# Harshs27/uGLAD

Measured on AMD Instinct MI355X. Metric: GLAD unroll-steps/sec (batch D×D Θ-updates), M=1024 D=128 L=30, higher is better.
Workload: dtype f32; 1 GPU; multi-task M=1024/GPU D=128 L=30 fp32 (BASELINE config 3; global batch 1024); pass=training step: forward + loss + backward + gradient exchange + Adam, sqrt_mode=ns10, parallelism=batch-sharded x1

## Files before the change

### uglad_amd/csrc/cell_bwd.h

```cpp
template <int NT>
__global__ __launch_bounds__(kThreads) void UGLAD_CELL_BWD_NAME(
    const float* __restrict__ Gnext, const float* __restrict__ S, const float* __restrict__ Zin,
    const float* __restrict__ half, const float* __restrict__ U, const float* __restrict__ beta,
    const float* __restrict__ lam_ptr, const float* __restrict__ params, float* __restrict__ Gout,
    float* __restrict__ grad_rho_partial, float* __restrict__ glam_partial, float* __restrict__ gws, int D, int mode,
#if UGLAD_CELL_BWD_GS
    int gs, int k_count, int lam_stride, float* __restrict__ gS) {
#else
    int gs, int k_count, int lam_stride) {
#endif
  constexpr int DP = NT * 32, LD = DP + 1;
  UGLAD_BIG_BUFFERS(sX, DP * LD, sY, DP * LD, gws)
  __shared__ float s_beta[DP], s_r[DP];
  __shared__ __attribute__((aligned(16))) float s_a0[DP], s_aN[DP];
  __shared__ float s_red[8];
  __shared__ float s_g[kWaves][kNRho + 1];
  const int tid = threadIdx.x, lane = tid & 63, w = tid >> 6;
  const size_t base = (size_t)blockIdx.x * D * D;
  const float* Sm = S + base;
  const float* Gm = Gnext + base;
  float* Go = Gout + base;
  const int grp = blockIdx.x / gs;
  params += (size_t)grp * kNParam;
  const size_t step_mdd = (size_t)gridDim.x * D * D, step_md = (size_t)gridDim.x * D;
  float g[kNRho];
#pragma unroll
  for (int q = 0; q < kNRho; ++q) g[q] = 0.f;
  constexpr int kMaxQ = ((DP / 2) * (DP + 1) + kThreads - 1) / kThreads;
  constexpr bool kPre = DP <= 128;
  constexpr int kQ = kPre ? kMaxQ : 8;
  constexpr int kIShift = kPre ? 8 : 16, kJMask = (1 << kIShift) - 1;
  const int D1 = D + 1, total = ((D + 1) / 2) * D1;
  const int sp = kThreads / D1, sc = kThreads - sp * D1;
  auto entry = [&](int e, int p, int c) -> int {
    if (e >= total) return -1;
    if (c < D - p) return (p << kIShift) | (p + c);
    const int i = D - 1 - p;
    return (i == p) ? -1 : ((i << kIShift) | (i + (c - (D - p))));
  };
  auto advance = [&](int& p, int& c) {
    c += sc;
    p += sp;
    if (c >= D1) {
      c -= D1;
      ++p;
    }
  };
  __shared__ unsigned short s_ent[kPre ? kMaxQ : 1][kPre ? kThreads : 1];
  if constexpr (kPre) {
    int p = tid / D1, c = tid - p * D1;
    for (int q = 0; q < kMaxQ; ++q) {
      s_ent[q][tid] = (unsigned short)entry(tid + kThreads * q, p, c);
      advance(p, c);
    }
  }
#pragma unroll 1
  for (int s = 0; s < k_count; ++s) {
    const bool first = (s == 0), last = (s == k_count - 1);
    const int tid = opaque_v(threadIdx.x), lane = tid & 63;
    const int w = __builtin_amdgcn_readfirstlane(tid >> 6);
    const float* Zm = Zin + base - s * step_mdd;
    const float* Hm = half + base - s * step_mdd;
    const float* Um = U + base - s * step_mdd;
    const float* bm = beta + (size_t)blockIdx.x * D - s * step_md;
    const float lam = lam_ptr[(long)grp - (long)s * lam_stride];
    const float c4 = 4.0f / lam, inv_lam2 = 1.0f / (lam * lam);

    KSTAMP(0);
    constexpr int kV4 = DP * DP / 4, kC4 = DP / 4;
    constexpr bool kFull4 = kV4 % (8 * kThreads) == 0, kFull1 = (DP * DP) % (8 * kThreads) == 0;
    const bool vec16 = (D == DP) && (((reinterpret_cast<size_t>(U) | (first ? reinterpret_cast<size_t>(Gnext) : 0)) & 15) == 0);
    if (vec16) {
      if (first) {
        for (int v0 = 0; v0 < kV4; v0 += 8 * kThreads) {
          f4 u[8], gv[8];
#pragma unroll
          for (int q = 0; q < 8; ++q) {
            const int idx = v0 + q * kThreads + tid;
            const unsigned at = (kFull4 || idx < kV4) ? 16u * idx : 0u;
            u[q] = load_at<f4>(Um, at);
            gv[q] = load_at<f4>(Gm, at);
          }
#pragma unroll
          for (int q = 0; q < 8; ++q) {
            const int idx = v0 + q * kThreads + tid;
            if (kFull4 || idx < kV4) {
              const int i = idx / kC4, k = 4 * (idx - i * kC4);
              sX[i * LD + k] = u[q].x, sX[i * LD + k + 1] = u[q].y, sX[i * LD + k + 2] = u[q].z, sX[i * LD + k + 3] = u[q].w;
              sY[i * LD + k] = gv[q].x, sY[i * LD + k + 1] = gv[q].y, sY[i * LD + k + 2] = gv[q].z, sY[i * LD + k + 3] = gv[q].w;
            }
          }
        }
      } else {
        for (int v0 = 0; v0 < kV4; v0 += 8 * kThreads) {
          f4 u[8];
#pragma unroll
          for (int q = 0; q < 8; ++q) {
            const int idx = v0 + q * kThreads + tid;
            u[q] = load_at<f4>(Um, (kFull4 || idx < kV4) ? 16u * idx : 0u);
          }
#pragma unroll
          for (int q = 0; q < 8; ++q) {
            const int idx = v0 + q * kThreads + tid;
            if (kFull4 || idx < kV4) {
              const int i = idx / kC4, k = 4 * (idx - i * kC4);
              sX[i * LD + k] = u[q].x, sX[i * LD + k + 1] = u[q].y, sX[i * LD + k + 2] = u[q].z, sX[i * LD + k + 3] = u[q].w;
            }
          }
        }
      }
    } else {
      constexpr int si = kThreads / DP, sk = kThreads - si * DP;
      int i = tid / DP, k = tid - i * DP;
      int off = i * D + k;
      const int soff = si * D + sk, wrap = D - DP;
      if (first) {
        for (int idx0 = 0; idx0 < DP * DP; idx0 += 8 * kThreads) {
          float u[8], gv[8];
          int dst[8];
          bool in[8];
#pragma unroll
          for (int q = 0; q < 8; ++q) {
            in[q] = (kFull1 || idx0 + q * kThreads + tid < DP * DP) && i < D && k < D;
            const unsigned at = in[q] ? 4u * off : 0u;
            u[q] = load_at<float>(Um, at);
            gv[q] = load_at<float>(Gm, at);
            dst[q] = i * LD + k;
            i += si, k += sk, off += soff;
            if (k >= DP) k -= DP, ++i, off += wrap;
          }
          __builtin_amdgcn_sched_barrier(0);
#pragma unroll
          for (int q = 0; q < 8; ++q) {
            if (kFull1 || idx0 + q * kThreads + tid < DP * DP) {
              sX[dst[q]] = in[q] ? u[q] : 0.f;
              sY[dst[q]] = in[q] ? gv[q] : 0.f;
            }
          }
        }
      } else {
        for (int idx0 = 0; idx0 < DP * DP; idx0 += 8 * kThreads) {
          float u[8];
          int dst[8];
          bool in[8];
#pragma unroll
          for (int q = 0; q < 8; ++q) {
            in[q] = (kFull1 || idx0 + q * kThreads + tid < DP * DP) && i < D && k < D;
            u[q] = load_at<float>(Um, in[q] ? 4u * off : 0u);
            dst[q] = i * LD + k;
            i += si, k += sk, off += soff;
            if (k >= DP) k -= DP, ++i, off += wrap;
          }
          __builtin_amdgcn_sched_barrier(0);
#pragma unroll
          for (int q = 0; q < 8; ++q) {
            if (kFull1 || idx0 + q * kThreads + tid < DP * DP) sX[dst[q]] = in[q] ? u[q] : 0.f;
          }
        }
      }
    }
    float a2 = 0.f;
    if (tid < D) {
      const float be = bm[tid];
      const float al = fmaf(be, be, c4);
      a2 = al * al;
    }
    const float nrmA = sqrtf(block_sum(a2, s_red));
    float r2 = 0.f;
    if (tid < DP) {
      float be = 0.f, r = 1.f;
      if (tid < D) {
        be = bm[tid];
        r = sqrt_spectrum(be, c4, nrmA, mode);
        r2 = r * r;
      }
      s_beta[tid] = be;
      s_r[tid] = r;
    }
    const float nrmR = sqrtf(block_sum(r2, s_red));
    if (mode == UGLAD_SQRT_NS10 && tid < DP) {
      float a = s_r[tid] / nrmR;
      s_a0[tid] = a;
#pragma unroll
      for (int it = 0; it < kNsIters; ++it) a = 0.5f * a * (3.f - a * a);
      s_aN[tid] = a;
    }
    __syncthreads();

    KSTAMP(1);
    using TU = Tiles<NT, true>;
    [[maybe_unused]] const int p0 = tid / D1, c0 = tid - p0 * D1;
    float gz[kQ];
    {
      [[maybe_unused]] int p = p0, c = c0;
      for (int q0 = 0; q0 < kMaxQ; q0 += kQ) {
        int pk[kQ];
        float hx[kQ], zz[kQ], gn[kQ], sv[kQ];
        if constexpr (kPre) {
#pragma unroll
          for (int u = 0; u < kQ; ++u) pk[u] = (int)(short)s_ent[u][tid];
          float gt[kQ];
#pragma unroll
          for (int u = 0; u < kQ; ++u) {
            const int i = pk[u] >> kIShift, j = pk[u] & kJMask;
            const bool in = pk[u] >= 0;
            const unsigned at = in ? 4u * ((unsigned)i * (unsigned)D + (unsigned)j) : 0u;
            gz[u] = 0.f;
            hx[u] = load_at<float>(Hm, at);
            zz[u] = load_at<float>(Zm, at);
            sv[u] = load_at<float>(Sm, at);
            gn[u] = sY[opaque_v(in ? i * LD + j : 0)];
            gt[u] = sY[opaque_v(in ? j * LD + i : 0)];
          }
#pragma unroll
          for (int u = 0; u < kQ; ++u) {
            const int i = pk[u] >> kIShift, j = pk[u] & kJMask;
            const bool in = pk[u] >= 0;
            hx[u] = in ? hx[u] : 0.f;
            zz[u] = in ? zz[u] : 0.f;
            sv[u] = in ? sv[u] : 0.f;
            gn[u] = in ? ((i == j) ? gn[u] : 0.5f * (gn[u] + gt[u])) : 0.f;
          }
        } else {
#pragma unroll
          for (int u = 0; u < kQ; ++u) {
            pk[u] = (q0 + u < kMaxQ) ? entry(tid + kThreads * (q0 + u), p, c) : -1;
            advance(p, c);
            const int i = pk[u] >> kIShift, j = pk[u] & kJMask;
            const bool in = pk[u] >= 0;
            hx[u] = in ? Hm[i * D + j] : 0.f;
            zz[u] = in ? Zm[i * D + j] : 0.f;
            sv[u] = in ? Sm[i * D + j] : 0.f;
            gn[u] = in ? ((i == j) ? sY[i * LD + j] : 0.5f * (sY[i * LD + j] + sY[j * LD + i])) : 0.f;
          }
        }
        constexpr int kQ2 = (kQ + 1) / 2;
#pragma unroll
        for (int h = 0; h < kQ2; ++h) {
          const int u0 = 2 * h, u1 = (2 * h + 1 < kQ) ? 2 * h + 1 : 2 * h;
          const bool has1 = 2 * h + 1 < kQ;
          if (!has1 && pk[u0] < 0) continue;
          RhoAct2 act2;
          rho_forward2(params, (v2f){hx[u0], has1 ? hx[u1] : 0.f}, (v2f){sv[u0], has1 ? sv[u1] : 0.f},
                       (v2f){zz[u0], has1 ? zz[u1] : 0.f}, act2);
#pragma unroll
          for (int c2 = 0; c2 < 2; ++c2) {
            const int u = c2 ? u1 : u0;
            if ((c2 == 0 || has1) && pk[u] >= 0) {
              const int i = pk[u] >> kIShift, j = pk[u] & kJMask;
              const RhoAct act = act2.half(c2);
              const float x = hx[u];
              const bool active = fabsf(x) > act.rho;
              const float sgn = (x > 0.f) ? 1.f : ((x < 0.f) ? -1.f : 0.f);
              const float g_rho = active ? -sgn * gn[u] : 0.f;
              float gx1, gx3;
              rho_backward(params, x, sv[u], zz[u], act, g_rho, (i == j) ? 1.f : 2.f, g, gx1, gx3);
#if UGLAD_CELL_BWD_GS
              gS[base + i * D + j] += rho_backward_col(params, act, g_rho, 1);
#endif
              const float gh = (active ? gn[u] : 0.f) + gx1;
              sY[i * LD + j] = gh;
              sY[j * LD + i] = gh;
              if (kPre) gz[u] = gx3;
              else Go[i * D + j] = gx3;
            }
          }
        }
      }
    }
    __syncthreads();

    KSTAMP(2);
    using T = Tiles<NT, false>;
    {
      f32x16 acc[T::kPerWave];
      gemm_lds<NT, false, false, false>(sY, sX, acc);
      __syncthreads();
      store_tiles<NT>(sY, acc);
    }
    __syncthreads();
    KSTAMP(3);
    float glam = 0.f;
    {
      f32x16 acc[TU::kPerWave];
      gemm_lds<NT, true, false, true>(sX, sY, acc);
      __syncthreads();
      KSTAMP(4);
#pragma unroll
      for (int n = 0; n < TU::kPerWave; ++n) {
        const int t = w + kWaves * n;
        if (t < TU::kCount) {
          int I, J;
          TU::ij(t, I, J);
          const int j = J * 32 + (lane & 31);
          const float a0j = s_a0[j], aNj = s_aN[j];
          const float rj = s_r[j], bj = s_beta[j];
          const float inv_2nrmR = 1.0f / (2.f * nrmR);
#pragma unroll
          for (int e4 = 0; e4 < 4; ++e4) {
            const int i0 = I * 32 + 8 * e4 + 4 * (lane >> 5);
            float Kr[4];
            if (mode == UGLAD_SQRT_EXACT) {
#pragma unroll
              for (int r = 0; r < 4; ++r) Kr[r] = 1.0f / (s_r[i0 + r] + rj);
            } else {
              const f4 a0 = *reinterpret_cast<const f4*>(&s_a0[i0]);
              const f4 aN = *reinterpret_cast<const f4*>(&s_aN[i0]);
              Kr[0] = ns_divided_difference(a0.x, a0j, aN.x, aNj, inv_2nrmR);
              Kr[1] = ns_divided_difference(a0.y, a0j, aN.y, aNj, inv_2nrmR);
              Kr[2] = ns_divided_difference(a0.z, a0j, aN.z, aNj, inv_2nrmR);
              Kr[3] = ns_divided_difference(a0.w, a0j, aN.w, aNj, inv_2nrmR);
            }
#pragma unroll
            for (int r = 0; r < 4; ++r) {
              const int e = 4 * e4 + r, i = i0 + r;
              if (I < J || i <= j) {
                float v = 0.f;
                if (i < D && j < D) {
                  const float K = Kr[r];
                  const float cij = acc[n][e];
                  if (i == j) glam = fmaf(cij, -2.f * K * inv_lam2, glam);
                  v = cij * 0.5f * fmaf(s_beta[i] + bj, K, -1.f);
                }
                sY[i * LD + j] = v;
                sY[j * LD + i] = v;
              }
            }
          }
        }
      }
    }
    __syncthreads();
    KSTAMP(5);
    {
      f32x16 acc[T::kPerWave];
      gemm_lds<NT, false, false, false>(sX, sY, acc);
      __syncthreads();
      store_tiles<NT>(sY, acc);
    }
    __syncthreads();
    KSTAMP(6);
    {
      f32x16 acc[TU::kPerWave];
      gemm_lds<NT, false, true, true>(sY, sX, acc);
      KSTAMP(7);
      __syncthreads();
#pragma unroll
      for (int n = 0; n < TU::kPerWave; ++n) {
        const int t = w + kWaves * n;
        if (t < TU::kCount) {
          int I, J;
          TU::ij(t, I, J);
#pragma unroll
          for (int e = 0; e < 16; ++e) sY[(I * 32 + acc_row(e, lane)) * LD + J * 32 + (lane & 31)] = acc[n][e];
        }
      }
    }
    __syncthreads();
    KSTAMP(20);
    {
      [[maybe_unused]] int p = p0, c = c0;
      for (int q0 = 0; q0 < kMaxQ; q0 += kQ) {
        int pk[kQ];
        float gb[kQ], sij[kQ];
#pragma unroll
        for (int u = 0; u < kQ; ++u) {
          if constexpr (kPre) {
            pk[u] = (int)(short)s_ent[u][tid];
          } else {
            pk[u] = (q0 + u < kMaxQ) ? entry(tid + kThreads * (q0 + u), p, c) : -1;
            advance(p, c);
          }
          const bool in = pk[u] >= 0;
          const int i = pk[u] >> kIShift, j = pk[u] & kJMask;
          gb[u] = sY[in ? i * LD + j : 0];
          sij[u] = load_at<float>(Sm, in ? 4u * ((unsigned)i * (unsigned)D + (unsigned)j) : 0u);
        }
        if (kPre) {
#pragma unroll
          for (int u = 0; u < kQ; ++u) {
            const bool in = pk[u] >= 0;
            const int i = pk[u] >> kIShift, j = pk[u] & kJMask;
            const float o = gz[u] - gb[u];
            sY[in ? i * LD + j : DP] = o;
            sY[in ? j * LD + i : DP] = o;
            glam = fmaf(in ? -sij[u] * inv_lam2 * ((i == j) ? 1.f : 2.f) : 0.f, gb[u], glam);
          }
        } else {
#pragma unroll
          for (int u = 0; u < kQ; ++u) {
            if (pk[u] >= 0) {
              const int i = pk[u] >> kIShift, j = pk[u] & kJMask;
              const float o = Go[i * D + j] - gb[u];
              sY[i * LD + j] = o;
              sY[j * LD + i] = o;
              glam = fmaf(-sij[u] * inv_lam2 * ((i == j) ? 1.f : 2.f), gb[u], glam);
            }
          }
        }
#if UGLAD_CELL_BWD_GS
        {
          const float inv_lam = 1.0f / lam;
#pragma unroll
          for (int u = 0; u < kQ; ++u) {
            if (pk[u] >= 0) {
              const int i = pk[u] >> kIShift, j = pk[u] & kJMask;
              const float v = fmaf(gb[u], inv_lam, gS[base + i * D + j]);
              gS[base + i * D + j] = v;
              gS[base + j * D + i] = v;
            }
          }
        }
#endif
      }
    }
    __syncthreads();
    KSTAMP(21);
    if (last) {
      const int si = kThreads / D, sj = kThreads - si * D;
      int i = tid / D, j = tid - i * D;
      for (int idx = tid; idx < D * D; idx += kThreads) {
        Go[idx] = sY[i * LD + j];
        j += sj;
        i += si;
        if (j >= D) {
          j -= D;
          ++i;
        }
      }
    }
    KSTAMP(8);
    if (last) {
#pragma unroll
      for (int q = 0; q < kNRho; ++q) {
        const float v = wave_sum(g[q]);
        if (lane == 0) s_g[w][q] = v;
      }
    }
    {
      const float v = wave_sum(glam);
      if (lane == 0) s_g[w][kNRho] = v;
    }
    __syncthreads();
    if (tid == kNRho || (last && tid < kNRho)) {
      float v = 0.f;
#pragma unroll
      for (int ww = 0; ww < kWaves; ++ww) v += s_g[ww][tid];
      if (tid < kNRho)
        grad_rho_partial[(size_t)blockIdx.x * kNRho + tid] += v;
      else
        (glam_partial - (size_t)s * gridDim.x)[blockIdx.x] = v;
    }
    KSTAMP(9);
  }
}
```

### uglad_amd/csrc/glad_device.h

```cpp
#pragma once
#include <hip/hip_runtime.h>

namespace uglad {

#ifndef UGLAD_THREADS
#define UGLAD_THREADS 512
#endif
constexpr int kThreads = UGLAD_THREADS;
constexpr int kWaves = kThreads / 64;
constexpr int kNsIters = 10;

constexpr int P_T = 0, P_RW1 = 1, P_RB1 = 10, P_RW2 = 13, P_RB2 = 22, P_RW3 = 25, P_RB3 = 28;
constexpr int P_LW1 = 29, P_LB1 = 35, P_LW2 = 38, P_LB2 = 41;
constexpr int kNParam = 42, kNRho = 28;

typedef float f32x16 __attribute__((ext_vector_type(16)));
struct alignas(16) f4 {
  float x, y, z, w;
};

#ifdef UGLAD_SIMT_EMUL
#define UGLAD_WAVE_SYNC() simt::wave_sync_point()
#else
#define UGLAD_WAVE_SYNC() asm volatile("s_waitcnt vmcnt(0) lgkmcnt(0)" ::: "memory")
#endif

template <int CTRL, int ROW_MASK = 0xf, int BANK_MASK = 0xf>
__device__ __forceinline__ float dpp_move(float v) {
  return __int_as_float(__builtin_amdgcn_update_dpp(0, __float_as_int(v), CTRL, ROW_MASK, BANK_MASK, false));
}

__device__ __forceinline__ float lane_xor1(float v) { return dpp_move<0xb1>(v); }

__device__ __forceinline__ float sum_halves(float v) {
#ifdef UGLAD_SIMT_EMUL
  return v + __shfl_xor(v, 32);
#else
  const auto r = __builtin_amdgcn_permlane32_swap(__float_as_uint(v), __float_as_uint(v), false, false);
  return __uint_as_float(r[0]) + __uint_as_float(r[1]);
#endif
}

__device__ __forceinline__ int opaque_v(int v) {
#ifndef UGLAD_SIMT_EMUL
  asm volatile("" : "+v"(v));
#endif
  return v;
}

template <typename T>
__device__ __forceinline__ T load_at(const float* __restrict__ base, unsigned bytes) {
  return *reinterpret_cast<const T*>(reinterpret_cast<const char*>(base) + bytes);
}

__device__ __forceinline__ float opaque_f(float v) {
#ifndef UGLAD_SIMT_EMUL
  asm volatile("" : "+v"(v));
#endif
  return v;
}

__device__ __forceinline__ int lane_now() {
#ifdef UGLAD_SIMT_EMUL
  return threadIdx.x & 63;
#else
  int l;
  asm volatile("v_mbcnt_lo_u32_b32 %0, -1, 0\n\tv_mbcnt_hi_u32_b32 %0, -1, %0" : "=v"(l));
  return l;
#endif
}

__device__ __forceinline__ float bcast_lane(float v, int src) {
  return __int_as_float(__builtin_amdgcn_readlane(__float_as_int(v), src));
}

__device__ __forceinline__ float wave_sum(float v) {
  v += dpp_move<0xb1>(v);
  v += dpp_move<0x4e>(v);
  v += dpp_move<0x124>(v);
  v += dpp_move<0x128>(v);
  v += dpp_move<0x142, 0xa>(v);
  v += dpp_move<0x143, 0xc>(v);
  return __int_as_float(__builtin_amdgcn_readlane(__float_as_int(v), 63));
}

__device__ __forceinline__ float block_sum(float v, float* s_red) {
  v = wave_sum(v);
  const int lane = threadIdx.x & 63, w = threadIdx.x >> 6;
  if (lane == 0) s_red[w] = v;
  __syncthreads();
  float t = 0.f;
#pragma unroll
  for (int i = 0; i < kWaves; ++i) t += s_red[i];
  __syncthreads();
  return t;
}

__device__ __forceinline__ float exp_acc(float x) {
  const float t = x * 1.44269504f;
  float e = fmaf(x, 1.44269504f, -t);
  e = fmaf(x, 1.925963033e-8f, e);
  const float r = __builtin_amdgcn_exp2f(t);
  return fmaf(r, e * 0.69314718f, r);
}

__device__ __forceinline__ float div_acc(float a, float b) {
  float q = __builtin_amdgcn_rcpf(b);
  q = fmaf(q, fmaf(-b, q, 1.0f), q);
  return a * q;
}

__device__ __forceinline__ float sigmoidf_(float x) {
  const float t = exp_acc(-fabsf(x));
  const float s = div_acc(1.0f, 1.0f + t);
  return (x >= 0.f) ? s : 1.0f - s;
}

__device__ __forceinline__ float tanhf_(float x) {
  const float t = exp_acc(-2.0f * fabsf(x));
  return copysignf(div_acc(1.0f - t, 1.0f + t), x);
}

struct RhoAct {
  float h1[3], h2[3], rho;
};

__device__ __forceinline__ void rho_forward(const float* __restrict__ p, float x1, float x2, float x3, RhoAct& a) {
#pragma unroll
  for (int o = 0; o < 3; ++o)
    a.h1[o] = tanhf_(fmaf(p[P_RW1 + 3 * o], x1, fmaf(p[P_RW1 + 3 * o + 1], x2, fmaf(p[P_RW1 + 3 * o + 2], x3, p[P_RB1 + o]))));
#pragma unroll
  for (int o = 0; o < 3; ++o)
    a.h2[o] = tanhf_(fmaf(p[P_RW2 + 3 * o], a.h1[0], fmaf(p[P_RW2 + 3 * o + 1], a.h1[1], fmaf(p[P_RW2 + 3 * o + 2], a.h1[2], p[P_RB2 + o]))));
  a.rho = sigmoidf_(fmaf(p[P_RW3], a.h2[0], fmaf(p[P_RW3 + 1], a.h2[1], fmaf(p[P_RW3 + 2], a.h2[2], p[P_RB3]))));
}

typedef float v2f __attribute__((ext_vector_type(2)));
__device__ __forceinline__ v2f fma2(v2f a, v2f b, v2f c) { return __builtin_elementwise_fma(a, b, c); }
__device__ __forceinline__ v2f splat2(float a) { return (v2f){a, a}; }
__device__ __forceinline__ v2f exp_acc2(v2f x) {
  const v2f t = x * 1.44269504f;
  v2f e = fma2(x, splat2(1.44269504f), -t);
  e = fma2(x, splat2(1.925963033e-8f), e);
  const v2f r = {__builtin_amdgcn_exp2f(t.x), __builtin_amdgcn_exp2f(t.y)};
  return fma2(r, e * 0.69314718f, r);
}
__device__ __forceinline__ v2f div_acc2(v2f a, v2f b) {
  v2f q = {__builtin_amdgcn_rcpf(b.x), __builtin_amdgcn_rcpf(b.y)};
  q = fma2(q, fma2(-b, q, splat2(1.0f)), q);
  return a * q;
}
__device__ __forceinline__ v2f tanh2(v2f x) {
  const v2f t = exp_acc2(-2.0f * __builtin_elementwise_abs(x));
  const v2f r = div_acc2(1.0f - t, 1.0f + t);
  return (v2f){copysignf(r.x, x.x), copysignf(r.y, x.y)};
}
__device__ __forceinline__ v2f sigmoid2(v2f x) {
  const v2f t = exp_acc2(-__builtin_elementwise_abs(x));
  const v2f s = div_acc2(splat2(1.0f), 1.0f + t);
  return (v2f){(x.x >= 0.f) ? s.x : 1.0f - s.x, (x.y >= 0.f) ? s.y : 1.0f - s.y};
}
struct RhoAct2 {
  v2f h1[3], h2[3], rho;
  __device__ __forceinline__ RhoAct half(int c) const {
    RhoAct a;
#pragma unroll
    for (int o = 0; o < 3; ++o) {
      a.h1[o] = c ? h1[o].y : h1[o].x;
      a.h2[o] = c ? h2[o].y : h2[o].x;
    }
    a.rho = c ? rho.y : rho.x;
    return a;
  }
};
__device__ __forceinline__ void rho_forward2(const float* __restrict__ p, v2f x1, v2f x2, v2f x3, RhoAct2& a) {
#pragma unroll
  for (int o = 0; o < 3; ++o)
    a.h1[o] = tanh2(fma2(splat2(p[P_RW1 + 3 * o]), x1,
                         fma2(splat2(p[P_RW1 + 3 * o + 1]), x2, fma2(splat2(p[P_RW1 + 3 * o + 2]), x3, splat2(p[P_RB1 + o])))));
#pragma unroll
  for (int o = 0; o < 3; ++o)
    a.h2[o] = tanh2(fma2(splat2(p[P_RW2 + 3 * o]), a.h1[0],
                         fma2(splat2(p[P_RW2 + 3 * o + 1]), a.h1[1], fma2(splat2(p[P_RW2 + 3 * o + 2]), a.h1[2], splat2(p[P_RB2 + o])))));
  a.rho = sigmoid2(fma2(splat2(p[P_RW3]), a.h2[0], fma2(splat2(p[P_RW3 + 1]), a.h2[1], fma2(splat2(p[P_RW3 + 2]), a.h2[2], splat2(p[P_RB3])))));
}

__device__ __forceinline__ float soft_threshold(float x, float rho) {
  const float m = fabsf(x) - rho;
  return m > 0.f ? copysignf(m, x) : 0.f;
}

__device__ __forceinline__ void rho_backward(const float* __restrict__ p, float x1, float x2, float x3, const RhoAct& a,
                                             float g_rho, float w, float* g, float& gx1, float& gx3) {
  const float go = g_rho * a.rho * (1.f - a.rho);
  const float gow = go * w;
  float ga2[3], ga1[3];
#pragma unroll
  for (int h = 0; h < 3; ++h) {
    g[(P_RW3 - 1) + h] += gow * a.h2[h];
    ga2[h] = go * p[P_RW3 + h] * (1.f - a.h2[h] * a.h2[h]);
  }
  g[P_RB3 - 1] += gow;
#pragma unroll
  for (int o = 0; o < 3; ++o) {
    const float t = ga2[o] * w;
#pragma unroll
    for (int h = 0; h < 3; ++h) g[(P_RW2 - 1) + 3 * o + h] += t * a.h1[h];
    g[(P_RB2 - 1) + o] += t;
  }
#pragma unroll
  for (int h = 0; h < 3; ++h) {
    const float s = ga2[0] * p[P_RW2 + h] + ga2[1] * p[P_RW2 + 3 + h] + ga2[2] * p[P_RW2 + 6 + h];
    ga1[h] = s * (1.f - a.h1[h] * a.h1[h]);
  }
#pragma unroll
  for (int o = 0; o < 3; ++o) {
    const float t = ga1[o] * w;
    g[(P_RW1 - 1) + 3 * o + 0] += t * x1;
    g[(P_RW1 - 1) + 3 * o + 1] += t * x2;
    g[(P_RW1 - 1) + 3 * o + 2] += t * x3;
    g[(P_RB1 - 1) + o] += t;
  }
  gx1 = ga1[0] * p[P_RW1 + 0] + ga1[1] * p[P_RW1 + 3] + ga1[2] * p[P_RW1 + 6];
  gx3 = ga1[0] * p[P_RW1 + 2] + ga1[1] * p[P_RW1 + 5] + ga1[2] * p[P_RW1 + 8];
}

__device__ __forceinline__ float rho_backward_col(const float* __restrict__ p, const RhoAct& a, float g_rho, int col) {
  const float go = g_rho * a.rho * (1.f - a.rho);
  float ga2[3], ga1[3];
#pragma unroll
  for (int h = 0; h < 3; ++h) ga2[h] = go * p[P_RW3 + h] * (1.f - a.h2[h] * a.h2[h]);
#pragma unroll
  for (int h = 0; h < 3; ++h) {
    const float s = ga2[0] * p[P_RW2 + h] + ga2[1] * p[P_RW2 + 3 + h] + ga2[2] * p[P_RW2 + 6 + h];
    ga1[h] = s * (1.f - a.h1[h] * a.h1[h]);
  }
  return ga1[0] * p[P_RW1 + col] + ga1[1] * p[P_RW1 + 3 + col] + ga1[2] * p[P_RW1 + 6 + col];
}

__device__ __forceinline__ void rho_backward2(const float* __restrict__ p, v2f x1, v2f x2, v2f x3, const RhoAct2& a, v2f g_rho,
                                              v2f w, v2f* g2, v2f& gx1, v2f& gx3) {
  const v2f go = g_rho * a.rho * (1.f - a.rho);
  const v2f gow = go * w;
  v2f ga2[3], ga1[3];
#pragma unroll
  for (int h = 0; h < 3; ++h) {
    g2[(P_RW3 - 1) + h] = fma2(gow, a.h2[h], g2[(P_RW3 - 1) + h]);
    ga2[h] = go * p[P_RW3 + h] * (1.f - a.h2[h] * a.h2[h]);
  }
  g2[P_RB3 - 1] += gow;
#pragma unroll
  for (int o = 0; o < 3; ++o) {
    const v2f t = ga2[o] * w;
#pragma unroll
    for (int h = 0; h < 3; ++h) g2[(P_RW2 - 1) + 3 * o + h] = fma2(t, a.h1[h], g2[(P_RW2 - 1) + 3 * o + h]);
    g2[(P_RB2 - 1) + o] += t;
  }
#pragma unroll
  for (int h = 0; h < 3; ++h) {
    const v2f s = ga2[0] * p[P_RW2 + h] + ga2[1] * p[P_RW2 + 3 + h] + ga2[2] * p[P_RW2 + 6 + h];
    ga1[h] = s * (1.f - a.h1[h] * a.h1[h]);
  }
#pragma unroll
  for (int o = 0; o < 3; ++o) {
    const v2f t = ga1[o] * w;
    g2[(P_RW1 - 1) + 3 * o + 0] = fma2(t, x1, g2[(P_RW1 - 1) + 3 * o + 0]);
    g2[(P_RW1 - 1) + 3 * o + 1] = fma2(t, x2, g2[(P_RW1 - 1) + 3 * o + 1]);
    g2[(P_RW1 - 1) + 3 * o + 2] = fma2(t, x3, g2[(P_RW1 - 1) + 3 * o + 2]);
    g2[(P_RB1 - 1) + o] += t;
  }
  gx1 = ga1[0] * p[P_RW1 + 0] + ga1[1] * p[P_RW1 + 3] + ga1[2] * p[P_RW1 + 6];
  gx3 = ga1[0] * p[P_RW1 + 2] + ga1[1] * p[P_RW1 + 5] + ga1[2] * p[P_RW1 + 8];
}

__device__ __forceinline__ float lambda_forward(const float* __restrict__ p, float n, float lam_prev) {
  float o = p[P_LB2];
#pragma unroll
  for (int h = 0; h < 3; ++h)
    o = fmaf(p[P_LW2 + h], tanhf(fmaf(p[P_LW1 + 2 * h], n, fmaf(p[P_LW1 + 2 * h + 1], lam_prev, p[P_LB1 + h]))), o);
  return sigmoidf_(o);
}

__device__ __forceinline__ float sqrt_spectrum(float beta, float c, float nrmA, int mode) {
  const float alpha = fmaf(beta, beta, c);
  if (mode == 0) return sqrtf(alpha);
  float y = alpha / nrmA, z = 1.f;
#pragma unroll
  for (int it = 0; it < kNsIters; ++it) {
    const float T = 0.5f * (3.f - z * y);
    y = y * T;
    z = T * z;
  }
  return y * sqrtf(nrmA);
}

__device__ __forceinline__ float ns_divided_difference(float a0_i, float a0_j, float aN_i, float aN_j, float inv_2nrmR) {
  return div_acc(aN_i + aN_j, a0_i + a0_j) * inv_2nrmR;
}

__device__ __forceinline__ float shifted_spectrum(float be, int D, float lam, int mode, double* __restrict__ s3, float& alpha,
                                                  float& cond) {
  const int tid = threadIdx.x;
  const double c4 = 4.0 / (double)lam, b = (double)be;
  const double al = b * b + c4;
  const double r_exact = sqrt(al);
  if (tid < D) {
    s3[tid] = al * al;
    s3[D + tid] = 0.5 * (r_exact - b) * b;
    s3[2 * D + tid] = b * b;
  }
  __syncthreads();
  double* part = s3 + 3 * D;
  if ((tid >> 6) == 0) {
    const double* a = s3 + ((tid >> 4) < 3 ? (tid >> 4) : 2) * D;
    double s = 0.0, mx = 0.0, mn = 1e300;
    for (int i = tid & 15; i < D; i += 16) {
      const double v = a[i];
      s += v;
      mx = v > mx ? v : mx;
      mn = v < mn ? v : mn;
    }
#pragma unroll
    for (int o = 1; o < 16; o *= 2) {
      s += __shfl_xor(s, o);
      const double mxo = __shfl_xor(mx, o), mno = __shfl_xor(mn, o);
      mx = mxo > mx ? mxo : mx;
      mn = mno < mn ? mno : mn;
    }
    if ((tid & 15) == 0 && tid < 48) part[tid >> 4] = s;
    if (tid == 32) {
      part[3] = mx;
      part[4] = mn;
    }
  }
  __syncthreads();
  const double n2 = part[0], pb = part[1], bb = part[2], b2max = part[3], b2min = part[4];
  cond = (float)((b2max + c4) / (b2min + c4));
  double a_opt = (bb > 0.0) ? -pb / bb : 0.0;
  a_opt = a_opt < 0.0 ? 0.0 : (a_opt > 1.0 ? 1.0 : a_opt);
  alpha = (float)a_opt;
  double r = r_exact;
  if (mode != 0) {
    const double nrmA = sqrt(n2);
    double y = al / nrmA, z = 1.0;
#pragma unroll
    for (int it = 0; it < kNsIters; ++it) {
      const double T = 0.5 * (3.0 - z * y);
      y = y * T;
      z = T * z;
    }
    r = y * sqrt(nrmA);
  }
  const double psi = 0.5 * (r - b) + (double)alpha * b;
  __syncthreads();
  return (tid < D) ? (float)psi : 0.f;
}

template <int DP>
__device__ __forceinline__ void pair_of(int r, int k, int& i1, int& i2) {
  constexpr int m = DP - 1;
  if (k == 0) {
    i1 = m;
    i2 = r;
  } else {
    i1 = r + k;
    if (i1 >= m) i1 -= m;
    i2 = r + m - k;
    if (i2 >= m) i2 -= m;
  }
}

template <int DP>
__device__ void jacobi_eig(float* __restrict__ A, float* __restrict__ V, float* s_t, float* s_s, float* s_h, float* s_red,
                           int* s_flag) {
  constexpr int LD = DP + 1, H = DP / 2;
  const int tid = threadIdx.x;
  float fro = 0.f;
  for (int idx = tid; idx < DP * DP; idx += kThreads) {
    const float v = A[(idx / DP) * LD + (idx % DP)];
    fro = fmaf(v, v, fro);
  }
  fro = sqrtf(block_sum(fro, s_red));
  const float thresh = 1e-8f * fro;
  for (int sweep = 0; sweep < 16; ++sweep) {
    if (tid == 0) *s_flag = 0;
    __syncthreads();
    for (int r = 0; r < DP - 1; ++r) {
      if (tid < H) {
        int p, q;
        pair_of<DP>(r, tid, p, q);
        const float apq = A[p * LD + q];
        float t = 0.f, s = 0.f, h = 0.f;
        if (fabsf(apq) > thresh) {
          const float app = A[p * LD + p], aqq = A[q * LD + q];
          const float tau = (aqq - app) / (2.f * apq);
          t = copysignf(1.f, tau) / (fabsf(tau) + sqrtf(fmaf(tau, tau, 1.f)));
          const float c = 1.f / sqrtf(fmaf(t, t, 1.f));
          s = t * c;
          h = s / (1.f + c);
          *s_flag = 1;
        }
        s_t[tid] = t;
        s_s[tid] = s;
        s_h[tid] = h;
      }
      __syncthreads();
      for (int b = tid; b < H * H; b += kThreads) {
        const int kr = b / H, kc = b - kr * H;
        int r1, r2, c1, c2;
        pair_of<DP>(r, kr, r1, r2);
        pair_of<DP>(r, kc, c1, c2);
        const float x11 = A[r1 * LD + c1], x12 = A[r1 * LD + c2], x21 = A[r2 * LD + c1], x22 = A[r2 * LD + c2];
        float z11, z12, z21, z22;
        if (kr == kc) {
          const float t = s_t[kr];
          z11 = x11 - t * x12;
          z22 = x22 + t * x12;
          z12 = (t != 0.f) ? 0.f : x12;
          z21 = (t != 0.f) ? 0.f : x21;
        } else {
          const float sr = s_s[kr], hr = s_h[kr], sc = s_s[kc], hc = s_h[kc];
          const float y11 = x11 - sr * (x21 + hr * x11), y21 = x21 + sr * (x11 - hr * x21);
          const float y12 = x12 - sr * (x22 + hr * x12), y22 = x22 + sr * (x12 - hr * x22);
          z11 = y11 - sc * (y12 + hc * y11);
          z12 = y12 + sc * (y11 - hc * y12);
          z21 = y21 - sc * (y22 + hc * y21);
          z22 = y22 + sc * (y21 - hc * y22);
        }
        A[r1 * LD + c1] = z11;
        A[r1 * LD + c2] = z12;
        A[r2 * LD + c1] = z21;
        A[r2 * LD + c2] = z22;
      }
      for (int b = tid; b < DP * H; b += kThreads) {
        const int i = b / H, kc = b - i * H;
        int c1, c2;
        pair_of<DP>(r, kc, c1, c2);
        const float sc = s_s[kc], hc = s_h[kc];
        const float v1 = V[i * LD + c1], v2 = V[i * LD + c2];
        V[i * LD + c1] = v1 - sc * (v2 + hc * v1);
        V[i * LD + c2] = v2 + sc * (v1 - hc * v2);
      }
      __syncthreads();
    }
    if (*s_flag == 0) break;
    __syncthreads();
  }
  __syncthreads();
}

template <int NT, bool UPPER>
struct Tiles {
  static constexpr int kCount = UPPER ? NT * (NT + 1) / 2 : NT * NT;
  static constexpr int kPerWave = (kCount + kWaves - 1) / kWaves;
  __device__ static __forceinline__ void ij(int t, int& I, int& J) {
    if (UPPER) {
      int i = 0, rem = t;
      while (rem >= NT - i) {
        rem -= NT - i;
        ++i;
      }
      I = i;
      J = i + rem;
    } else {
      I = t / NT;
      J = t - I * NT;
    }
  }
};

__device__ __forceinline__ int acc_row(int reg, int lane) { return (reg & 3) + 8 * (reg >> 2) + 4 * (lane >> 5); }

__device__ __forceinline__ void mfma_tile(const float* __restrict__ Ap, int a_si, int a_sk, const float* __restrict__ Bp,
                                          int b_sk, int b_sj, int K, f32x16& acc) {
  const int lane = opaque_v(threadIdx.x) & 63, li = lane & 31, kh = lane >> 5;
  const float* a = Ap + li * a_si + kh * a_sk;
  const float* b = Bp + li * b_sj + kh * b_sk;
  float a0[8], b0[8], a1[8], b1[8];
#pragma unroll
  for (int u = 0; u < 8; ++u) {
    a0[u] = a[2 * u * a_sk];
    b0[u] = b[2 * u * b_sk];
  }
  for (int k = 0; k < K; k += 16) {
    const bool more = k + 16 < K;
    const float* an = a + (more ? 16 * a_sk : 0);
    const float* bn = b + (more ? 16 * b_sk : 0);
#pragma unroll
    for (int u = 0; u < 8; ++u) {
      a1[u] = an[2 * u * a_sk];
      b1[u] = bn[2 * u * b_sk];
    }
#pragma unroll
    for (int u = 0; u < 8; ++u) acc = __builtin_amdgcn_mfma_f32_32x32x2f32(a0[u], b0[u], acc, 0, 0, 0);
#pragma unroll
    for (int u = 0; u < 8; ++u) {
      a0[u] = a1[u];
      b0[u] = b1[u];
    }
    a = an;
    b = bn;
  }
}

#if defined(UGLAD_BF16X3) && !defined(UGLAD_SIMT_EMUL)
#include "../../scripts/retired/bf16x3_tile.h"
#define UGLAD_GEMM_TILE mfma_tile_bf16x3
#else
#define UGLAD_GEMM_TILE mfma_tile
#endif

template <int NT, bool TA, bool TB, bool UPPER>
__device__ __forceinline__ void gemm_lds(const float* __restrict__ X, const float* __restrict__ Y,
                                         f32x16 (&acc)[Tiles<NT, UPPER>::kPerWave]) {
  constexpr int DP = NT * 32, LD = DP + 1;
  using T = Tiles<NT, UPPER>;
  const int w = __builtin_amdgcn_readfirstlane(opaque_v(threadIdx.x) >> 6);
#pragma unroll
  for (int n = 0; n < T::kPerWave; ++n) {
    const int t = w + kWaves * n;
#pragma unroll
    for (int e = 0; e < 16; ++e) acc[n][e] = 0.f;
    if (t < T::kCount) {
      int I, J;
      T::ij(t, I, J);
      UGLAD_GEMM_TILE(TA ? X + I * 32 : X + I * 32 * LD, TA ? 1 : LD, TA ? LD : 1, TB ? Y + J * 32 * LD : Y + J * 32,
                      TB ? 1 : LD, TB ? LD : 1, DP, acc[n]);
    }
  }
}

template <int NT>
__device__ __forceinline__ void store_tiles(float* __restrict__ Y, const f32x16 (&acc)[Tiles<NT, false>::kPerWave]) {
  constexpr int LD = NT * 32 + 1;
  using T = Tiles<NT, false>;
  const int tid = opaque_v(threadIdx.x), lane = tid & 63, w = __builtin_amdgcn_readfirstlane(tid >> 6);
#pragma unroll
  for (int n = 0; n < T::kPerWave; ++n) {
    const int t = w + kWaves * n;
    if (t < T::kCount) {
      int I, J;
      T::ij(t, I, J);
#pragma unroll
      for (int e = 0; e < 16; ++e) Y[(I * 32 + acc_row(e, lane)) * LD + J * 32 + (lane & 31)] = acc[n][e];
    }
  }
}

#ifdef UGLAD_STAMPS
__device__ unsigned long long g_cwg[4096][3];
__device__ unsigned long long g_lstamps[4][96];
__device__ unsigned long long g_kstamps[32];
#define KSTAMP(i) do { if (threadIdx.x == 0 && blockIdx.x == 0) g_kstamps[i] = __builtin_amdgcn_s_memtime(); } while (0)
#define UGLAD_STAMP(ws, i) do { if (threadIdx.x == 0 && (i) < 64) (ws).stamp[i] = __builtin_amdgcn_s_memtime(); } while (0)
#elif defined(UGLAD_PHASE_EXIT)
__device__ int g_exit_at;
#define KSTAMP(i) do { if (g_exit_at == 100 + (i)) __builtin_amdgcn_endpgm(); } while (0)
#define UGLAD_STAMP(ws, i) do { if (g_exit_at == (i)) __builtin_amdgcn_endpgm(); } while (0)
#else
#define KSTAMP(i) do {} while (0)
#define UGLAD_STAMP(ws, i) do {} while (0)
#endif

__device__ __forceinline__ void copy_out_matrix(float* __restrict__ dst, const float* __restrict__ src, int D, int LD) {
  const int tid = threadIdx.x;
  if (((D & 3) == 0) && ((reinterpret_cast<size_t>(dst) & 15) == 0)) {
    const int D4 = D >> 2;
    for (int idx = tid; idx < D * D4; idx += kThreads) {
      const int i = idx / D4, j = 4 * (idx - i * D4);
      const float* p = src + i * LD + j;
      f4 v = {p[0], p[1], p[2], p[3]};
      *reinterpret_cast<f4*>(dst + (size_t)i * D + j) = v;
    }
  } else {
    const int si = kThreads / D, sj = kThreads - si * D;
    int i = tid / D, j = tid - i * D;
    for (int idx = tid; idx < D * D; idx += kThreads) {
      dst[idx] = src[i * LD + j];
      j += sj;
      i += si;
      if (j >= D) {
        j -= D;
        ++i;
      }
    }
  }
}

template <int DP>
constexpr int kTfacFloats = (DP / 32) * 1024;
template <int DP>
constexpr int kWsPerMatrix = 3 * DP + kTfacFloats<DP>;
template <int DP>
constexpr int big_floats() {
  return 2 * ((DP * (DP + 1) + 3) & ~3);
}
#define UGLAD_BIG_BUFFERS(A, NA, B, NB, GWS)                                                                     \
  constexpr bool kGM = DP > 128;                                                                                 \
  __shared__ __attribute__((aligned(16))) float A##_lds[kGM ? 4 : (NA)];                                         \
  __shared__ __attribute__((aligned(16))) float B##_lds[kGM ? 4 : (NB)];                                         \
  float* A = kGM ? (GWS) + (size_t)gridDim.x * kWsPerMatrix<DP> + (size_t)blockIdx.x * big_floats<DP>() : A##_lds; \
  float* B = kGM ? A + big_floats<DP>() / 2 : B##_lds;

template <int DP>
__device__ __forceinline__ float* tfac_behind_flags(float* ws, int M, int m) {
  static_assert(kTfacFloats<DP> / 2 >= 4, "flags and packed T factors outgrow the T region: M + 3 <= M kTfacFloats / 2 needs kTfacFloats / 2 >= 4");
  return ws + (size_t)M * 3 * DP + ((M + 3) & ~3) + (size_t)m * (kTfacFloats<DP> / 2);
}

}
```

Measured before the change: 1.305 million unroll-steps/s.

## Pack rho backward into v2f pairs and prefetch H/Z/S before spectrum reductions

```diff
diff --git a/uglad_amd/csrc/cell_bwd.h b/uglad_amd/csrc/cell_bwd.h
--- a/uglad_amd/csrc/cell_bwd.h
+++ b/uglad_amd/csrc/cell_bwd.h
@@ -23,9 +23,11 @@
   const int grp = blockIdx.x / gs;
   params += (size_t)grp * kNParam;
   const size_t step_mdd = (size_t)gridDim.x * D * D, step_md = (size_t)gridDim.x * D;
+  constexpr bool kPackA = NT <= 7;
   float g[kNRho];
-#pragma unroll
-  for (int q = 0; q < kNRho; ++q) g[q] = 0.f;
+  [[maybe_unused]] v2f g2[kNRho];
+#pragma unroll
+  for (int q = 0; q < kNRho; ++q) g[q] = 0.f, g2[q] = splat2(0.f);
   constexpr int kMaxQ = ((DP / 2) * (DP + 1) + kThreads - 1) / kThreads;
   constexpr bool kPre = DP <= 128;
   constexpr int kQ = kPre ? kMaxQ : 8;
@@ -159,9 +161,23 @@
         }
       }
     }
+    const float be_ld = load_at<float>(bm, (tid < D) ? 4u * (unsigned)tid : 0u);
+    [[maybe_unused]] float hx_a[kQ], zz_a[kQ], sv_a[kQ];
+    if constexpr (kPre) {
+      int ea[kQ];
+#pragma unroll
+      for (int u = 0; u < kQ; ++u) ea[u] = (int)(short)s_ent[u][tid];
+#pragma unroll
+      for (int u = 0; u < kQ; ++u) {
+        const unsigned at = (unsigned)opaque_v((ea[u] >= 0) ? 4 * ((ea[u] >> kIShift) * D + (ea[u] & kJMask)) : 0);
+        hx_a[u] = load_at<float>(Hm, at);
+        zz_a[u] = load_at<float>(Zm, at);
+        sv_a[u] = load_at<float>(Sm, at);
+      }
+    }
     float a2 = 0.f;
     if (tid < D) {
-      const float be = bm[tid];
+      const float be = be_ld;
       const float al = fmaf(be, be, c4);
       a2 = al * al;
     }
@@ -170,7 +186,7 @@
     if (tid < DP) {
       float be = 0.f, r = 1.f;
       if (tid < D) {
-        be = bm[tid];
+        be = be_ld;
         r = sqrt_spectrum(be, c4, nrmA, mode);
         r2 = r * r;
       }
@@ -204,22 +220,15 @@
           for (int u = 0; u < kQ; ++u) {
             const int i = pk[u] >> kIShift, j = pk[u] & kJMask;
             const bool in = pk[u] >= 0;
-            const unsigned at = in ? 4u * ((unsigned)i * (unsigned)D + (unsigned)j) : 0u;
-            gz[u] = 0.f;
-            hx[u] = load_at<float>(Hm, at);
-            zz[u] = load_at<float>(Zm, at);
-            sv[u] = load_at<float>(Sm, at);
             gn[u] = sY[opaque_v(in ? i * LD + j : 0)];
             gt[u] = sY[opaque_v(in ? j * LD + i : 0)];
           }
+          static_assert(kPackA || !kPre, "the tabled entries go with the packed backward");
 #pragma unroll
           for (int u = 0; u < kQ; ++u) {
             const int i = pk[u] >> kIShift, j = pk[u] & kJMask;
-            const bool in = pk[u] >= 0;
-            hx[u] = in ? hx[u] : 0.f;
-            zz[u] = in ? zz[u] : 0.f;
-            sv[u] = in ? sv[u] : 0.f;
-            gn[u] = in ? ((i == j) ? gn[u] : 0.5f * (gn[u] + gt[u])) : 0.f;
+            hx[u] = hx_a[u], zz[u] = zz_a[u], sv[u] = sv_a[u];
+            gn[u] = (i == j) ? gn[u] : 0.5f * (gn[u] + gt[u]);
           }
         } else {
 #pragma unroll
@@ -235,6 +244,49 @@
           }
         }
         constexpr int kQ2 = (kQ + 1) / 2;
+        if constexpr (kPackA) {
+          [[maybe_unused]] const int tid_a = opaque_v(tid);
+#pragma unroll
+          for (int h = 0; h < kQ2; ++h) {
+            const int u0 = 2 * h, u1 = (2 * h + 1 < kQ) ? 2 * h + 1 : 2 * h;
+            const bool has1 = 2 * h + 1 < kQ;
+            const int e0 = kPre ? (int)(short)s_ent[kPre ? u0 : 0][kPre ? tid_a : 0] : pk[u0];
+            const int e1 = kPre ? (int)(short)s_ent[kPre ? u1 : 0][kPre ? tid_a : 0] : pk[u1];
+            const bool in0 = e0 >= 0, in1 = has1 && e1 >= 0;
+            const int i0 = e0 >> kIShift, j0 = e0 & kJMask, i1 = e1 >> kIShift, j1 = e1 & kJMask;
+            const v2f x = {hx[u0], has1 ? hx[u1] : 0.f}, s2 = {sv[u0], has1 ? sv[u1] : 0.f}, z2 = {zz[u0], has1 ? zz[u1] : 0.f};
+            const v2f gn2 = {gn[u0], has1 ? gn[u1] : 0.f};
+            RhoAct2 act2;
+            rho_forward2(params, x, s2, z2, act2);
+            const bool on0 = in0 && fabsf(x.x) > act2.rho.x, on1 = in1 && fabsf(x.y) > act2.rho.y;
+            const v2f gact = {on0 ? gn2.x : 0.f, on1 ? gn2.y : 0.f};
+            const v2f g_rho = {on0 ? ((x.x > 0.f) ? -gn2.x : gn2.x) : 0.f, on1 ? ((x.y > 0.f) ? -gn2.y : gn2.y) : 0.f};
+            const v2f wgt = {on0 ? ((i0 == j0) ? 1.f : 2.f) : 0.f, on1 ? ((i1 == j1) ? 1.f : 2.f) : 0.f};
+            v2f gx1, gx3;
+            rho_backward2(params, x, s2, z2, act2, g_rho, wgt, g2, gx1, gx3);
+#pragma unroll
+            for (int q = 0; q < kNRho; ++q) g2[q] = opaque_f2(g2[q]);
+            gx3 = opaque_f2(gx3);
+#if UGLAD_CELL_BWD_GS
+            if (in0) gS[base + i0 * D + j0] += rho_backward_col(params, act2.half(0), g_rho.x, 1);
+            if (in1) gS[base + i1 * D + j1] += rho_backward_col(params, act2.half(1), g_rho.y, 1);
+#endif
+            const v2f gh = gact + gx1;
+            sY[opaque_v(in0 ? i0 * LD + j0 : DP)] = gh.x;
+            sY[opaque_v(in0 ? j0 * LD + i0 : DP)] = gh.x;
+            if (has1) {
+              sY[opaque_v(in1 ? i1 * LD + j1 : DP)] = gh.y;
+              sY[opaque_v(in1 ? j1 * LD + i1 : DP)] = gh.y;
+            }
+            if constexpr (kPre) {
+              gz[u0] = gx3.x;
+              if (has1) gz[u1] = gx3.y;
+            } else {
+              if (in0) Go[i0 * D + j0] = gx3.x;
+              if (in1) Go[i1 * D + j1] = gx3.y;
+            }
+          }
+        } else {
 #pragma unroll
         for (int h = 0; h < kQ2; ++h) {
           const int u0 = 2 * h, u1 = (2 * h + 1 < kQ) ? 2 * h + 1 : 2 * h;
@@ -266,6 +318,7 @@
             }
           }
         }
+        }
       }
     }
     __syncthreads();
@@ -433,6 +486,7 @@
     if (last) {
 #pragma unroll
       for (int q = 0; q < kNRho; ++q) {
+        if constexpr (kPackA) g[q] = g2[q].x + g2[q].y;
         const float v = wave_sum(g[q]);
         if (lane == 0) s_g[w][q] = v;
       }
diff --git a/uglad_amd/csrc/glad_device.h b/uglad_amd/csrc/glad_device.h
--- a/uglad_amd/csrc/glad_device.h
+++ b/uglad_amd/csrc/glad_device.h
@@ -136,6 +136,12 @@
 }
 
 typedef float v2f __attribute__((ext_vector_type(2)));
+__device__ __forceinline__ v2f opaque_f2(v2f v) {
+#ifndef UGLAD_SIMT_EMUL
+  asm volatile("" : "+v"(v));
+#endif
+  return v;
+}
 __device__ __forceinline__ v2f fma2(v2f a, v2f b, v2f c) { return __builtin_elementwise_fma(a, b, c); }
 __device__ __forceinline__ v2f splat2(float a) { return (v2f){a, a}; }
 __device__ __forceinline__ v2f exp_acc2(v2f x) {
@@ -258,7 +264,8 @@
   }
 #pragma unroll
   for (int h = 0; h < 3; ++h) {
-    const v2f s = ga2[0] * p[P_RW2 + h] + ga2[1] * p[P_RW2 + 3 + h] + ga2[2] * p[P_RW2 + 6 + h];
+    const v2f s = (h == 0) ? fma2(ga2[2], splat2(p[P_RW2 + 6]), fma2(ga2[0], splat2(p[P_RW2]), ga2[1] * p[P_RW2 + 3]))
+                           : fma2(ga2[2], splat2(p[P_RW2 + 6 + h]), fma2(ga2[1], splat2(p[P_RW2 + 3 + h]), ga2[0] * p[P_RW2 + h]));
     ga1[h] = s * (1.f - a.h1[h] * a.h1[h]);
   }
 #pragma unroll
@@ -269,8 +276,8 @@
     g2[(P_RW1 - 1) + 3 * o + 2] = fma2(t, x3, g2[(P_RW1 - 1) + 3 * o + 2]);
     g2[(P_RB1 - 1) + o] += t;
   }
-  gx1 = ga1[0] * p[P_RW1 + 0] + ga1[1] * p[P_RW1 + 3] + ga1[2] * p[P_RW1 + 6];
-  gx3 = ga1[0] * p[P_RW1 + 2] + ga1[1] * p[P_RW1 + 5] + ga1[2] * p[P_RW1 + 8];
+  gx1 = fma2(ga1[2], splat2(p[P_RW1 + 6]), fma2(ga1[0], splat2(p[P_RW1 + 0]), ga1[1] * p[P_RW1 + 3]));
+  gx3 = opaque_f2(ga1[2] * p[P_RW1 + 8]) + fma2(ga1[1], splat2(p[P_RW1 + 5]), ga1[0] * p[P_RW1 + 2]);
 }
 
 __device__ __forceinline__ float lambda_forward(const float* __restrict__ p, float n, float lam_prev) {
```

Measured after the change: 1.325 million unroll-steps/s, median of 6. 1.02x the previous value.
